# Matthew-Mosior/text-compression

Measured on AMD Instinct MI355X. Metric: BWT+MTF+RLE encode MB/s on 1 GiB ACGTN, higher is better.
Workload: dtype u8; 1 GPU; 1 x 1073741824-byte iid ACGTN record(s) (splitmix64 counter generator), fused BWT->MTF->RLE encode, in/out resident in HBM; record_bytes=1073741824, records=1, parallelism=record-per-gpu x1

## Files before the change

text-compression_amd/csrc/tc_msd.hpp:

```cpp
#pragma once
#include "tc_sa.hpp"

#ifndef MSD_NT
#define MSD_NT 1024
#endif
#ifndef MSD_ITEMS
#define MSD_ITEMS 8
#endif
#define MSD_TILE (MSD_NT * MSD_ITEMS)
#ifndef MSD_GROUP
#define MSD_GROUP 16
#endif
#define MSD_GLOG (MSD_GROUP == 32 ? 5 : MSD_GROUP == 16 ? 4 : 3)
#ifndef MSD_SUB
#define MSD_SUB 1
#endif
#ifndef MSD_BPC
#define MSD_BPC 1
#endif
#define MSD_LEVELS 3
#define MSDF_CAP_SMALL 2048
#ifndef MSDF_KO_NT
#define MSDF_KO_NT 256
#endif
// ... 274 lines not shown
                add(k0); add(k1); add(k2); add(k3);
            }
            for (; p < hi; p += MSD_NT) add(keys[p]);
        }
        __syncthreads();
        if (JOINT) {
            for (u32 w = tid; w < 32768; w += MSD_NT) {
                const u32 v = s_joint[w];
                if (v) {
                    atomicAdd(&joint_out[((size_t)sq * 256 + jr.dig[w >> 8]) * 256 + (w & 255u)], v);
                    atomicAdd(&s_cnt[jr.dig[w >> 8]], v);
                    s_joint[w] = 0;
                }
            }
            __syncthreads();
        }
        if (tid < 256) {
            L.seg[((size_t)sq + b) * 256 + tid] = s_cnt[tid];
            s_cnt[tid] = 0;
        }
    }
}

__global__ __launch_bounds__(256) void msd_scan_kernel(MsdLevel L, u32 G, u32 *maxchild) {
    __shared__ u32 s_scan[256 / 64 + 1];
    const u32 q = blockIdx.x, d = threadIdx.x;
    const u32 cnt = L.pcnt[q];
    const size_t c = (size_t)q * 256 + d;
    if (cnt == 0) {
        L.ccnt[c] = 0;
        L.cstart[c] = L.pstart[q];
        return;
    }
    if (L.aligned) {
        const u32 tot = L.cnt_in[c];
        u32 all;
        const u32 excl = block_excl_sum<256>(tot, s_scan, &all);
        const u32 start = L.pstart[q] + excl;
        L.cstart[c] = start;
        L.ccnt[c] = tot;
        L.seg[((size_t)q + msd_block_of_parent(L, q, G)) * 256 + d] = start;
        if (d == 0 && all != cnt) atomicOr(L.flags, 8u);
        if (maxchild) {
            u32 m = tot;
#pragma unroll
            for (int x = 32; x >= 1; x >>= 1) {
                const u32 o = __shfl_xor(m, x, 64);
                m = m > o ? m : o;
            }
            if ((d & 63) == 0 && m > MSDF_CAP_SMALL) atomicMax(maxchild, m);
        }
        return;
    }
    const u32 T = L.tpre[L.nparents];
    const u32 bf = msd_block_of_tile(T, L.tpre[q], G), bl = msd_block_of_tile(T, L.tpre[q + 1] - 1, G);
    u32 tot = 0;
#pragma unroll 8
    for (u32 b = bf; b <= bl; b++) {
        const u32 v = L.seg[((size_t)q + b) * 256 + d];
        tot += msd_tile_lo(T, b, G) < msd_tile_lo(T, b + 1, G) ? v : 0u;
    }
    u32 all;
    const u32 excl = block_excl_sum<256>(tot, s_scan, &all);
    u32 run = L.pstart[q] + excl;
    L.cstart[c] = run;
    L.ccnt[c] = tot;
#pragma unroll 8
    for (u32 b = bf; b <= bl; b++) {
        const size_t o = ((size_t)q + b) * 256 + d;
        const u32 v = L.seg[o];
        if (msd_tile_lo(T, b, G) >= msd_tile_lo(T, b + 1, G)) continue;
        L.seg[o] = run;
        run += v;
    }
    if (maxchild) {
        u32 m = tot;
#pragma unroll
        for (int x = 32; x >= 1; x >>= 1) {
            const u32 o = __shfl_xor(m, x, 64);
            m = m > o ? m : o;
        }
        if ((d & 63) == 0 && m > MSDF_CAP_SMALL) atomicMax(maxchild, m);
    }
}

typedef u32 msd_u32x4 __attribute__((ext_vector_type(4)));
template <bool KEYGEN, bool VALS = true>
__global__ __launch_bounds__(MSD_NT) void msd_partition_kernel(MsdLevel L, const u64 *kin, const u32 *vin,
                                                               u64 *kout, u32 *vout, const u8 *text,
                                                               RadixKeyGen kg) {
    __shared__ __attribute__((aligned(16))) u64 s_keys[MSD_TILE];
    __shared__ __attribute__((aligned(16))) u32 s_vals[VALS ? MSD_TILE : 4];
    __shared__ __attribute__((aligned(16))) u64 c_keys[256 * MSD_GROUP];
    __shared__ __attribute__((aligned(16))) u32 c_vals[VALS ? 256 * MSD_GROUP : 4];
    __shared__ u32 s_cnt[256 * MSD_SUB], s_dstart[256 * MSD_SUB], s_r[256], s_cur[256], s_ph[256];
    __shared__ u32 s_scan[16];
    __shared__ u64 s_lmask[4];
#ifdef MSD_PROFILE
    __shared__ u64 s_dbg[2];
    if (threadIdx.x == 0) { s_dbg[0] = 0; s_dbg[1] = 0; }
#endif
    __shared__ u16 s_live[256];
    __shared__ u16 s_klut[KEYGEN ? 256 : 1];
    constexpr bool KG_SPLIT = KEYGEN && !VALS && MSD_ITEMS == 8;
    __shared__ __attribute__((aligned(16))) u8 s_kr[KG_SPLIT ? MSD_TILE + 16 + 80 + 32 : 16];
    __shared__ __attribute__((aligned(16))) u8 s_kg8[KG_SPLIT ? MSD_TILE + 64 : 16];
    __shared__ u32 s_scan2[2];
    static_assert(MSD_GROUP == 8 || MSD_GROUP == 16 || MSD_GROUP == 32, "group = 8, 16 or 32 pairs");
    static_assert(((size_t)MSD_TILE * (VALS ? 12 : 8) + 256 * MSD_GROUP * (VALS ? 12 : 8) + 8192 + (KG_SPLIT ? 2 * MSD_TILE + 256 : 0)) * (VALS ? 1 : MSD_BPC) <= 163840, "LDS budget");
    __shared__ MsdTileInfo s_info[4];

    const u32 tid = threadIdx.x, G = gridDim.x, b = msd_logical_wg(blockIdx.x, G);
    if (KEYGEN && tid < 256) s_klut[tid] = kg.lut[tid];
    if (tid < 256) { s_r[tid] = 0; s_ph[tid] = 0; s_cur[tid] = 0; }
    for (u32 i = tid; i < 256 * MSD_SUB; i += MSD_NT) s_cnt[i] = 0;
    if (tid == 0) {
        u32 ta = 0, tb = 0;
        if (!(L.aligned && (*L.flags & 8u))) msd_block_range(L, b, G, &ta, &tb);
        s_scan2[0] = ta; s_scan2[1] = tb;
    }
    __syncthreads();
    const u32 t0 = s_scan2[0], t1 = s_scan2[1];
    if (t0 >= t1) return;
    MsdCur cs = {};
    if (tid == 0) {
        msd_cur_init(L, cs, t0);
        msd_cur_info(L, cs, t0, t1, &s_info[0]);
        msd_cur_info(L, cs, t0 + 1, t1, &s_info[1]);
        msd_cur_info(L, cs, t0 + 2, t1, &s_info[2]);
    }
    __syncthreads();

    constexpr int KG_PRE = 16, KG_SLOTS = MSD_TILE + KG_PRE + 80;
    u16 *k_c = reinterpret_cast<u16 *>(s_keys);
    u16 *k_g = k_c + KG_SLOTS;
    u8 *k_r = reinterpret_cast<u8 *>(k_g + KG_SLOTS);
    static_assert(KG_SLOTS * 5 <= MSD_TILE * 8, "key-generation image must fit under the staging keys");
    const u32 kg_units = KEYGEN ? (KG_PRE + MSD_TILE + kg.P * kg.s + kg.s + 15) / 16 : 0;

    u64 key[MSD_ITEMS];
    u32 val[MSD_ITEMS];
    msd_u32x4 raw = {0, 0, 0, 0}, nraw = {0, 0, 0, 0};
    auto kg_edge = [&](const MsdTileInfo ti) {
        return ti.base < (u32)KG_PRE || (u64)ti.base - KG_PRE + (u64)kg_units * 16 > (u64)kg.n_text ||
               ((((uintptr_t)text) + ti.base) & 15) != 0;
    };
    auto kg_load_plain = [&](const MsdTileInfo ti) {
        msd_u32x4 rw = {0, 0, 0, 0};
        if (tid < kg_units) {
            const i64 p0 = (i64)ti.base - KG_PRE + (i64)tid * 16;
            const i64 nt = (i64)kg.n_text;
            if (p0 >= 0 && p0 + 16 <= nt && ((((uintptr_t)text) + (u64)p0) & 15) == 0) {
                rw = *reinterpret_cast<const msd_u32x4 *>(text + p0);
            } else {
                u32 x[4] = {0, 0, 0, 0};
#pragma unroll 1
                for (int j = 0; j < 16; j++) {
                    const i64 pp = p0 + j;
                    const u32 c = (pp >= 0 && pp < nt) ? (u32)text[pp] : 0u;
                    x[j >> 2] |= c << (8 * (j & 3));
                }
                rw.x = x[0]; rw.y = x[1]; rw.z = x[2]; rw.w = x[3];
            }
        }
        return rw;
    };
// ... 933 lines not shown
```

text-compression_amd/csrc/tc_sa.hpp:

```cpp
#pragma once
#include <type_traits>
#include "tc_radix.hpp"

#define SA_NT 256
#define SA_ITEMS 16
#define SA_TILE (SA_NT * SA_ITEMS)
#define KB_HALO 72

struct SaConfig {
    u32 sigma_text;
    u32 B;
    u32 w;
    u32 s;
    u32 P;
    u32 h0;
    double entropy;
    u16 lut[256];
};

#ifdef __HIPCC__

__global__ __launch_bounds__(256) void hist256_kernel(const u8 *__restrict__ text, u64 n,
                                                      u32 *__restrict__ counts) {
    __shared__ u32 s_h[256 * 64];
// ... 899 lines not shown
            if (total == 0) return;
            if (l == 0) {
                abase = atomicAdd(&a.counters[0], total);
                atomicOr(&a.counters[1], 2u);
            }
            abase = __shfl(abase, 0, 64);
            if ((u64)abase + total > (u64)a.fix_cap) return;
        }
    }
}

__global__ __launch_bounds__(256) void finish_filter_kernel(u32 *__restrict__ slot, u32 count,
                                                            const u32 *__restrict__ ovbits, u32 *ndropped) {
    __shared__ u32 s_n;
    if (threadIdx.x == 0) s_n = 0;
    __syncthreads();
    u32 mine = 0;
    for (u64 k = (u64)blockIdx.x * 256 + threadIdx.x; k < count; k += (u64)gridDim.x * 256) {
        const u32 j = slot[k];
        if ((ovbits[j >> 5] >> (j & 31)) & 1u) {
            slot[k] = 0xFFFFFFFFu;
            mine++;
        }
    }
    for (int d = 32; d >= 1; d >>= 1) mine += (u32)__shfl_xor((int)mine, d, 64);
    if (lane_id() == 0 && mine) atomicAdd(&s_n, mine);
    __syncthreads();
    if (threadIdx.x == 0 && s_n) atomicAdd(ndropped, s_n);
}

__global__ __launch_bounds__(64) void finish_regions_kernel(const u32 *__restrict__ rcount, u32 rcap,
                                                            u32 *__restrict__ roff, u32 *__restrict__ counters) {
    const u32 l = threadIdx.x;
    const u32 c = rcount[l * FIN_RSTRIDE];
    const bool over = c > rcap;
    u32 inc = over ? rcap : c;
    const u32 mine = inc;
    for (int d = 1; d < 64; d <<= 1) {
        const u32 t = (u32)__shfl_up((int)inc, d, 64);
        if ((int)l >= d) inc += t;
    }
    roff[l] = inc - mine;
    const u64 anyover = __ballot(over);
    if (l == 63) {
        roff[64] = inc;
        counters[0] = anyover ? 0xFFFFFFF0u : inc;
    }
}
__global__ __launch_bounds__(256) void finish_compact_kernel(const u32 *__restrict__ roff, u32 rcap,
                                                             const u32 *__restrict__ in_slot,
                                                             const u32 *__restrict__ in_idx,
                                                             const u32 *__restrict__ in_grp,
                                                             u32 *__restrict__ out_slot, u32 *__restrict__ out_idx,
                                                             u32 *__restrict__ out_grp,
                                                             const u32 *__restrict__ in_x = nullptr, u32 *__restrict__ out_x = nullptr,
                                                             u32 x_cap = 0) {
    const u32 total = roff[64];
    for (u64 k = (u64)blockIdx.x * 256 + threadIdx.x; k < total; k += (u64)gridDim.x * 256) {
        u32 lo = 0, hi = FIN_REGIONS;
        while (hi - lo > 1) {
            const u32 mid = (lo + hi) >> 1;
            if (roff[mid] <= (u32)k) lo = mid; else hi = mid;
        }
        const u64 src = (u64)lo * rcap + ((u32)k - roff[lo]);
        out_slot[k] = in_slot[src];
        out_idx[k] = in_idx[src];
        out_grp[k] = in_grp[src];
        if (in_x && k < x_cap) out_x[k] = in_x[src];
    }
}

#define TP_SLOT_BITS 17
#define TP_BLOOM_LOG2 18
#define TP_MAX_TIED (1u << 15)
struct TiedTable {
    u64 *key;
    u32 *grp;
    u32 *cnt;
    u32 *bloom;
};
__device__ __forceinline__ u64 tp_mix(u64 v) { return v * 0x9E3779B97F4A7C15ull; }
__device__ __forceinline__ u32 tp_sym(u32 c) { return __umul24(c, 0x9E3779u); }
__device__ __forceinline__ u32 tp_rotl(u32 x, u32 r) { return __builtin_amdgcn_alignbit(x, x, (32u - r) & 31u); }

__global__ __launch_bounds__(256) void tied_table_kernel(const u32 *__restrict__ klo, const u32 *__restrict__ khi,
                                                         const u32 *__restrict__ grp, u32 m, u32 B, u32 sdig, u32 P,
                                                         TiedTable T) {
    const u32 k = blockIdx.x * 256 + threadIdx.x;
    if (k >= m) return;
    const u64 key56 = ((u64)khi[k] << 32) | klo[k];
    u64 v = 0;
    u32 H = 0;
    for (u32 f = 0; f < P; f++) {
        const u32 g = (u32)(key56 >> (48 - 8 * f)) & 255u;
        u32 div = 1;
        for (u32 j = 1; j < sdig; j++) div *= B;
        for (u32 j = 0; j < sdig; j++, div /= B) {
            const u32 c = (g / div) % B;
            v = v * B + c;
            H = tp_rotl(H, 1) ^ tp_sym(c);
        }
    }
    const u32 hb = H >> (32 - TP_BLOOM_LOG2);
    atomicOr(&T.bloom[hb >> 5], 1u << (hb & 31));
    u32 slot = (u32)(tp_mix(v) >> (64 - TP_SLOT_BITS));
    for (u32 probe = 0; probe < (1u << TP_SLOT_BITS); probe++) {
        const u64 old = atomicCAS((unsigned long long *)&T.key[slot], 0ull, (unsigned long long)v);
        if (old == 0ull || old == v) {
            T.grp[slot] = grp[k];
            return;
        }
        slot = (slot + 1) & ((1u << TP_SLOT_BITS) - 1u);
    }
}

#define TPK_NT 256
#define TPK_PER 64
#define TPK_TILE (TPK_NT * TPK_PER)
#define TPK_PAD(p) ((p) + ((p) >> 6) * 4u)
template <int S>
__global__ __launch_bounds__(TPK_NT) void tied_probe_kernel(const u8 *__restrict__ text, u32 n, RadixKeyGen kg,
                                                            TiedTable T, u32 *__restrict__ out_slot,
                                                            u32 *__restrict__ out_idx, u32 *__restrict__ out_grp,
                                                            u32 *total, u32 cap) {
    constexpr u32 h = 7 * S;
    constexpr int WD = (64 + h + 3) / 4;
    static_assert(h <= 56 && WD <= 30, "the window is 16 own dwords + at most 14 of the next thread's");
    __shared__ u32 s_bloom[(1u << TP_BLOOM_LOG2) / 32];
    __shared__ __attribute__((aligned(16))) u8 s_code[TPK_PAD(TPK_TILE + 64) + 16];
    __shared__ u8 s_lut[256];
    const u32 tid = threadIdx.x;
    const u32 B = kg.B;
    for (u32 i = tid; i < (1u << TP_BLOOM_LOG2) / 32; i += TPK_NT) s_bloom[i] = T.bloom[i];
    s_lut[tid] = (u8)kg.lut[tid];
    const u32 ntiles = (n + TPK_TILE - 1) / TPK_TILE;
    constexpr int NU = (TPK_TILE + 64 + TPK_NT * 16 - 1) / (TPK_NT * 16);
    uint4 raw[NU];
    auto unit_ok = [&](u32 base, int i) -> bool {
        const u32 p = ((u32)i * TPK_NT + tid) * 16;
        const u64 g = (u64)base + p;
        return p < TPK_TILE + 64 && g + 16 <= n && ((((uintptr_t)text) + g) & 15) == 0;
    };
    auto fetch = [&](u32 base) {
#pragma unroll
        for (int i = 0; i < NU; i++) {
            raw[i] = make_uint4(0, 0, 0, 0);
            if (unit_ok(base, i)) raw[i] = *reinterpret_cast<const uint4 *>(text + (u64)base + ((u32)i * TPK_NT + tid) * 16);
        }
    };
    if (blockIdx.x < ntiles) fetch(blockIdx.x * TPK_TILE);
    for (u32 tile = blockIdx.x; tile < ntiles; tile += gridDim.x) {
        const u32 base = tile * TPK_TILE;
        __syncthreads();
#pragma unroll
        for (int i = 0; i < NU; i++) {
            const u32 p = ((u32)i * TPK_NT + tid) * 16;
            if (p >= TPK_TILE + 64) continue;
            const u64 g = (u64)base + p;
            if (unit_ok(base, i)) {
                const u32 x[4] = {raw[i].x, raw[i].y, raw[i].z, raw[i].w};
#pragma unroll
                for (int j = 0; j < 16; j++) s_code[TPK_PAD(p + j)] = s_lut[(x[j >> 2] >> (8 * (j & 3))) & 255u];
            } else {
                for (int j = 0; j < 16; j++) s_code[TPK_PAD(p + j)] = g + j < n ? s_lut[text[g + j]] : (u8)0;
            }
        }
        if (tile + gridDim.x < ntiles) fetch((tile + gridDim.x) * TPK_TILE);
        lds_barrier();
        const u32 p0 = tid * TPK_PER;
        if (base + p0 < n) {
            u32 W[WD];
            {
                const u32 *own = reinterpret_cast<const u32 *>(s_code + 68u * tid);
                const u32 *nxt = reinterpret_cast<const u32 *>(s_code + 68u * (tid + 1));
#pragma unroll
                for (int i = 0; i < WD; i++) W[i] = i < 16 ? own[i] : nxt[i - 16];
            }
            auto code = [&](int x) -> u32 { return (W[x >> 2] >> (8 * (x & 3))) & 255u; };
            u32 H = 0;
#pragma unroll
            for (int j = 0; j < (int)h; j++) H = tp_rotl(H, 1) ^ tp_sym(code(j));
            u64 hits = 0;
#pragma unroll
            for (int j = 0; j < TPK_PER; j++) {
                const u32 hb = H >> (32 - TP_BLOOM_LOG2);
                hits |= (u64)((s_bloom[hb >> 5] >> (hb & 31)) & 1u) << j;
                H = tp_rotl(H, 1) ^ tp_rotl(tp_sym(code(j)), h & 31u) ^ tp_sym(code(j + (int)h));
            }
            while (hits) {
                const u32 j = (u32)__builtin_ctzll(hits);
                hits &= hits - 1;
                const u32 pos = base + p0 + j;
                if (pos >= n) break;
                u64 v = 0;
                for (u32 x = 0; x < h; x++) v = v * B + s_code[TPK_PAD(p0 + j + x)];
                u32 slot = (u32)(tp_mix(v) >> (64 - TP_SLOT_BITS));
                for (u32 probe = 0; probe < (1u << TP_SLOT_BITS); probe++) {
                    const u64 kk = T.key[slot];
                    if (kk == v) {
                        const u32 jj = atomicAdd(&T.cnt[slot], 1u);
                        const u32 o = atomicAdd(total, 1u);
                        if (o < cap) {
                            const u32 g0 = T.grp[slot];
                            out_slot[o] = g0 + jj;
                            out_idx[o] = pos;
                            out_grp[o] = g0;
                        }
                        break;
                    }
                    if (kk == 0ull) break;
                    slot = (slot + 1) & ((1u << TP_SLOT_BITS) - 1u);
                }
            }
        }
    }
}

__global__ __launch_bounds__(256) void pack_active_kernel(const u32 *__restrict__ slot,
                                                          const u32 *__restrict__ grp, u32 m,
                                                          u64 *__restrict__ keys) {
    u32 k = blockIdx.x * 256 + threadIdx.x;
    if (k < m) keys[k] = ((u64)slot[k] << 32) | grp[k];
}
__global__ __launch_bounds__(256) void unpack_active_kernel(const u64 *__restrict__ keys, u32 m,
                                                            u32 *__restrict__ slot,
                                                            u32 *__restrict__ grp) {
    u32 k = blockIdx.x * 256 + threadIdx.x;
    if (k < m) {
        slot[k] = (u32)(keys[k] >> 32);
        grp[k] = (u32)keys[k];
    }
}

struct RankLookup {
    const u32 *isa;
    const u32 *t_idx;
    const u32 *t_rank;
    u32 t_n;
    const u64 *skeys;
    const u64 *tkeys;
    int tshift;
    const u32 *sa;
    const u64 *t_bits;
    const u32 *t_dir;
    const u32 *kdir;
    int kdir_bits;
    const u8 *text;
    u32 n, N;
    u32 B, w, s, P;
    u32 h0;
    u16 lut[256];
};

__device__ __forceinline__ int suffix_cmp(const u8 *text, u32 n, u64 x, u64 y, u32 h) {
    for (u32 t = 0; t < h; t++, x++, y++) {
        int cx = x < n ? (int)text[x] : -1, cy = y < n ? (int)text[y] : -1;
        if (cx != cy) return cx < cy ? -1 : 1;
        if (cx < 0) return 0;
    }
    return 0;
}

template <bool WAVE = false>
__device__ __forceinline__ u32 rank_of(const RankLookup &r, const u16 *s_lut, u64 p) {
    if (p >= r.N) return 0u;
    if (r.isa) return r.isa[p];
    if (r.t_bits) {
        const u64 wbits = r.t_bits[p >> 6];
        if ((wbits >> (p & 63)) & 1ull)
            return r.t_rank[r.t_dir[p >> 6] + (u32)__popcll(wbits & ((1ull << (p & 63)) - 1ull))];
    } else {
        u32 lo = 0, hi = r.t_n;
        while (lo < hi) {
            u32 mid = (lo + hi) >> 1;
            if (r.t_idx[mid] < (u32)p) lo = mid + 1; else hi = mid;
        }
        if (lo < r.t_n && r.t_idx[lo] == (u32)p) return r.t_rank[lo];
    }
    u64 key = 0;
    if (p + 64 <= r.n && r.P * r.s <= 56) {
        u64 wv[7];
#pragma unroll
        for (int x = 0; x < 7; x++) __builtin_memcpy(&wv[x], r.text + p + 8 * x, 8);
        const u32 len = r.P * r.s;
        int sh = 64;
        u32 g = 0, t = 0;
#pragma unroll
        for (int k = 0; k < 56; k++) {
            if ((u32)k < len) {
                g = g * r.B + (u32)s_lut[(u32)(wv[k >> 3] >> (8 * (k & 7))) & 255u];
                if (++t == r.s) {
                    sh -= (int)r.w;
                    key |= (u64)g << sh;
                    g = 0; t = 0;
                }
            }
// ... 338 lines not shown
```

text-compression_amd/csrc/tc_sa_host.hpp:

```cpp
#pragma once
#include <chrono>

#include "tc_sa_plan.hpp"

#ifndef SA_KDIR_BITS
#define SA_KDIR_BITS 26
#endif
struct SaBuffers {
    u64 *k0, *k1;
    u32 *v0, *v1;
    u32 *isa;
    u32 *v2;
    u32 *act[2][4];
    u64 *sk[2];
    u32 *sv[2];
    u32 *t_idx, *t_rank;
    u64 *t_bits;
    u32 *t_dir;
    u32 *t_bsum;
    u32 *fin_rc;
    u32 *kdir;
    u64 sparse_cap;
    u32 *hist;
    u64 *rstatus;
// ... 9 lines not shown
};

static inline u64 msd_min_n() { return (u64)env_int("TC_SA_MSD_MIN_LOG2", 27) >= 40 ? ~0ull : 1ull << env_int("TC_SA_MSD_MIN_LOG2", 27); }
static inline bool msd_wanted(u64 N) { return env_int("TC_SA_MSD", 1) != 0 && N >= msd_min_n() && N > 4 * MSD_TILE; }

static size_t sa_carve(Arena &A, u64 N, SaBuffers &b, bool own_v1) {
    b.k0 = A.get<u64>(N);
    b.k1 = A.get<u64>(N);
    b.v0 = A.get<u32>(N);
    b.v1 = own_v1 ? A.get<u32>(N) : nullptr;
    b.isa = A.get<u32>(N + 1);
    b.v2 = A.get<u32>(N);
    b.sparse_cap = N / 8 + 1024;
    for (int s = 0; s < 2; s++) {
        for (int q = 0; q < 3; q++) b.act[s][q] = A.get<u32>(N);
        b.act[s][3] = A.get<u32>(b.sparse_cap);
        b.sk[s] = A.get<u64>(b.sparse_cap);
        b.sv[s] = A.get<u32>(b.sparse_cap);
    }
    b.t_idx = A.get<u32>(b.sparse_cap);
    b.t_rank = A.get<u32>(b.sparse_cap);
    b.t_bits = A.get<u64>(N / 64 + 2);
    b.t_dir = A.get<u32>(N / 64 + 2);
    b.t_bsum = A.get<u32>(N / 64 / BDIR_TILE + 2);
    b.fin_rc = A.get<u32>(FIN_REGIONS * FIN_RSTRIDE + 128);
    b.kdir = A.get<u32>(((size_t)1 << SA_KDIR_BITS) + 2 + ((size_t)1 << SA_KDIR_BITS) / KDF_CHUNK + 64);
    b.hist = A.get<u32>(RDX_MAX_PASSES * RDX_BINS);
    b.rstatus = A.get<u64>(radix_status_words(N));
    b.gstatus = A.get<u64>(2 * (size_t)tc_cdiv(N, GRP_TILE) + 4);
    b.counts = A.get<u32>(260);
    {
        SegBuffers &g = b.seg;
        g.cap_runs = (size_t)(N / SEG_CAP + 2);
        g.cap_tiles = (size_t)(N / SEG_PT + 2) + g.cap_runs;
        g.segbits = A.get<u64>(seg_bit_words(N));
        g.ybits = A.get<u64>(seg_bit_words(N));
        for (int q = 0; q < 2; q++) {
            g.lstart[q] = A.get<u32>(g.cap_runs);
            g.lsize[q] = A.get<u32>(g.cap_runs);
            g.ltbase[q] = A.get<u32>(g.cap_runs);
            g.lshift[q] = A.get<u32>(g.cap_runs);
        }
        g.tile_seg = A.get<u32>(g.cap_tiles);
        g.hist = A.get<u32>(g.cap_runs * 256);
        g.mm = A.get<u32>(g.cap_runs * 2);
        g.counters = A.get<u32>(64);
    }
    for (int l = 0; l <= MSD_LEVELS; l++) b.msd_pstart[l] = b.msd_pcnt[l] = nullptr;
    if (msd_wanted(N)) {
        b.msd_grid = 256 * MSD_BPC;
        size_t np = 1;
        for (int l = 0; l <= MSD_LEVELS; l++, np *= 256) {
            b.msd_pstart[l] = A.get<u32>(np);
            b.msd_pcnt[l] = A.get<u32>(np);
            if (l < MSD_LEVELS) {
                b.msd_tpre[l] = A.get<u32>(np + 1);
                b.msd_seg[l] = A.get<u32>((np + b.msd_grid) * 256);
            }
        }
        b.msd_joint = A.get<u32>((size_t)256 * 256 * 256);
        b.tp.key = A.get<u64>((size_t)1 << TP_SLOT_BITS);
        b.tp.grp = A.get<u32>((size_t)1 << TP_SLOT_BITS);
        b.tp.cnt = A.get<u32>((size_t)1 << TP_SLOT_BITS);
        b.tp.bloom = A.get<u32>(((size_t)1 << TP_BLOOM_LOG2) / 32);
    }
    b.chain_ref = A.get<u32>(N + 1);
    b.chain_code = A.get<u32>(N + 1);
    b.chain_summ = A.get<u32>(chain_summ_words());
    return A.off;
}

enum SaSlot {
    SA_SLOT_PRIMARY = 0,
    SA_SLOT_ACTIVE = 1,
    SA_SLOT_PROBE = 11,
    SA_SLOT_TIED = 12,
    SA_SLOT_DROPPED = 13,
    SA_SLOT_SAMPLE = 14,
    SA_SLOT_MAXCHILD = 15,
    SA_SLOT_SEG = 24,
    SA_SLOT_ERR = 62,
    SA_SLOT_MSD_PROF = 64,
    SA_SLOT_MSDK_PROF = 112,
};
static inline u32 sa_slot_lo(const tc_ctx *ctx, int slot) { return (u32)(ctx->h_scalars[slot] & 0xffffffffu); }
static inline u32 sa_slot_hi(const tc_ctx *ctx, int slot) { return (u32)(ctx->h_scalars[slot] >> 32); }
static inline u32 *sa_dev_slot(tc_ctx *ctx, int slot) { return reinterpret_cast<u32 *>(ctx->d_scalars + slot); }

#ifdef SEG_PROFILE
static void seg_profile_dump(tc_ctx *ctx, u32 m) {
    u64 h[16];
    TC_HIP(ctx, hipStreamSynchronize(ctx->stream));
    TC_HIP(ctx, hipMemcpyFromSymbol(h, HIP_SYMBOL(seg_prof), sizeof h));
    const double w = (double)(h[7] | 1);
    fprintf(stderr, "seg_small: %llu members, %llu windows (that sort), mid members per window %.0f | cycles per window: bits %.0f attr+masks %.0f (prefix) %.0f image %.0f tiny+compact %.0f tiny store %.0f network %.0f store %.0f\n",
            (unsigned long long)m, (unsigned long long)h[7], h[8] / w, h[0] / w, h[1] / w, 0.0, h[2] / w, h[3] / w, h[4] / w, h[5] / w, h[6] / w);
    memset(h, 0, sizeof h);
    TC_HIP(ctx, hipMemcpyToSymbol(HIP_SYMBOL(seg_prof), h, sizeof h));
}
#else
static inline void seg_profile_dump(tc_ctx *, u32) {}
#endif

static void seg_sort_pairs(tc_ctx *ctx, SegBuffers &g, u64 *kx, u32 *vx, u64 *ky, u32 *vy, u32 m, int rbits) {
    hipStream_t s = ctx->stream;
    const u32 nwords = (u32)seg_bit_words(m);
    TC_HIP(ctx, hipMemsetAsync(g.ybits, 0, (size_t)nwords * sizeof(u64), s));
    TC_HIP(ctx, hipMemsetAsync(g.counters, 0, 8 * sizeof(u32), s));
    u32 igrid = tc_cdiv((u64)nwords * 64, 256);
    if (igrid > 16384) igrid = 16384;
    seg_init_kernel<<<igrid, 256, 0, s>>>(kx, m, g.segbits, nwords, g.lstart[0], g.lsize[0], g.ltbase[0], g.lshift[0],
                                          (u32)(rbits > 8 ? rbits - 8 : 0), g.counters, (u32)g.cap_runs);
    TC_LAUNCH_CHECK(ctx);
    const int nlev = 8;
    int cur = 0;
    for (int L = 0;; L++) {
        TC_HIP(ctx, hipMemcpyAsync(&ctx->h_scalars[SA_SLOT_SEG], g.counters + 2 * cur, 2 * sizeof(u32), hipMemcpyDeviceToHost, s));
        TC_HIP(ctx, hipStreamSynchronize(s));
        const u32 S = sa_slot_lo(ctx, SA_SLOT_SEG), T = sa_slot_hi(ctx, SA_SLOT_SEG);
        if (S == 0) break;
        if (L >= nlev) TC_FAIL(ctx, TC_ERR_INTERNAL, "segmented sort: %u runs still unsorted after %d levels", S, nlev);
        if (S > g.cap_runs || T > g.cap_tiles) TC_FAIL(ctx, TC_ERR_INTERNAL, "segmented sort: %u long runs / %u tiles exceed the tables", S, T);
        const int nxt = cur ^ 1;
        TC_HIP(ctx, hipMemsetAsync(g.hist, 0, (size_t)S * 256 * sizeof(u32), s));
        seg_mm_init_kernel<<<tc_cdiv(S, 256), 256, 0, s>>>(g.mm, S);
        TC_LAUNCH_CHECK(ctx);
        TC_HIP(ctx, hipMemsetAsync(g.counters + 2 * nxt, 0, 2 * sizeof(u32), s));
        u32 wgrid = tc_cdiv(S, 4);
        if (wgrid > 8192) wgrid = 8192;
        seg_tilemap_kernel<<<wgrid, 256, 0, s>>>(g.lsize[cur], g.ltbase[cur], S, g.tile_seg, (u32)g.cap_tiles);
        TC_LAUNCH_CHECK(ctx);
        seg_count_kernel<<<T, 256, 0, s>>>(kx, ky, g.lstart[cur], g.lsize[cur], g.ltbase[cur], g.lshift[cur], g.tile_seg, g.counters + 2 * cur, g.hist, g.mm);
        TC_LAUNCH_CHECK(ctx);
        seg_scan_kernel<<<wgrid, 256, 0, s>>>(g.lstart[cur], g.lsize[cur], g.lshift[cur], g.counters + 2 * cur, g.hist, g.mm, g.segbits, 0,
                                              g.lstart[nxt], g.lsize[nxt], g.ltbase[nxt], g.lshift[nxt], g.counters + 2 * nxt, (u32)g.cap_runs);
        TC_LAUNCH_CHECK(ctx);
        seg_scatter_kernel<<<T, 256, 0, s>>>(kx, vx, ky, vy, g.lstart[cur], g.lsize[cur], g.ltbase[cur], g.lshift[cur], g.tile_seg, g.counters + 2 * cur,
                                             g.hist, g.mm, g.ybits);
        TC_LAUNCH_CHECK(ctx);
        cur = nxt;
    }
    seg_small_kernel<<<tc_cdiv(m, SEG_SPAN), SEG_NT, 0, s>>>(kx, vx, ky, vy, m, g.segbits, g.ybits);
    TC_LAUNCH_CHECK(ctx);
    seg_profile_dump(ctx, m);
}

static void sa_choose_config(const u32 *counts, u64 n, int forced_fields, SaConfig &c) {
    u32 sig = 0;
    double H = 0;
    for (int v = 0; v < 256; v++) {
        c.lut[v] = 0;
        if (counts[v]) {
            c.lut[v] = (u16)(++sig);
            double p = (double)counts[v] / (double)n;
            H -= p * log2(p);
        }
    }
    c.sigma_text = sig;
    c.B = sig + 1;
    if (c.B <= 16) {
        c.w = 8;
        c.s = 1;
        u32 pw = c.B;
        while (pw * c.B <= 256) {
            pw *= c.B;
            c.s++;
// ... 336 lines not shown
    fa.ovbits = b.act[1][0];
    tc_memset_async(ctx, ctx->d_scalars + SA_SLOT_TIED, 0, 2 * sizeof(u64));
    tc_memset_async(ctx, b.fin_rc, 0, (FIN_REGIONS * FIN_RSTRIDE + 128) * sizeof(u32));
}

static Round0Out sa_round0_lsd(SaRun &R, const Round0Plan &pl) {
    Round0Out o;
    o.msd = o.msd_big = o.keyonly = false;
    sa_round0_begin(R, pl.topbits, o);
    R.st().msd_path = 0;
    RadixPlan plan;
    plan.add_range(64 - pl.topbits, 64);
    RadixBuffers rb = sa_build_keys_and_sort(R, plan, true);
    o.npass = plan.npass;
    o.keys = rb.keys;
    o.fa.keys = rb.keys; o.fa.sa_in = rb.vals;
    const u32 waves = tc_cdiv(R.N, 64 * FIN_WPW);
    finish_kernel<<<tc_cdiv(waves, FIN_NT / 64), FIN_NT, 0, R.stream()>>>(o.fa);
    TC_LAUNCH_CHECK(R.ctx);
    return o;
}

static Round0Out sa_round0_msd(SaRun &R, const Round0Plan &pl, bool keyonly) {
    tc_ctx *ctx = R.ctx;
    SaBuffers &b = R.b;
    const SaConfig &cfg = R.cfg;
    hipStream_t s = R.stream();
    tc_stats &st = R.st();
    const u32 n = (u32)R.n, N = (u32)R.N;
    Round0Out o;
    o.msd = true; o.msd_big = pl.msd_big; o.keyonly = keyonly;
    sa_round0_begin(R, 8 * MSD_LEVELS, o);
    u32 *counters = o.fa.counters;
    RadixKeyGen kg = sa_keygen(R);
    radix_keygen_hash(kg);
    if (R.K.keygen_hash == 0) kg.hash_ok = 0;
    MsdTextDigit td;
    sa_fill(cfg, td);
    td.text = R.text; td.n = n;
    td.hash_ok = kg.hash_ok; td.hsh = kg.hsh; td.tlo = kg.tlo; td.thi = kg.thi;
    u32 G = b.msd_grid < (u32)ctx->num_cus * MSD_BPC ? b.msd_grid : (u32)ctx->num_cus * MSD_BPC;
    if (ctx->reserved_cus > 0 && G > (u32)(ctx->num_cus - ctx->reserved_cus) * MSD_BPC)
        G = (u32)(ctx->num_cus - ctx->reserved_cus) * MSD_BPC;
    if (R.K.msd_grid > 0 && (u32)R.K.msd_grid < G) G = (u32)R.K.msd_grid;
    u32 *maxchild = sa_dev_slot(ctx, SA_SLOT_MAXCHILD);
    msd_root_kernel<<<1, 1, 0, s>>>(b.msd_pstart[0], b.msd_pcnt[0], N, maxchild);
    TC_LAUNCH_CHECK(ctx);
    u64 *kbuf[2] = {b.k0, b.k1};
    u32 *vbuf[2] = {keyonly ? nullptr : b.v0, keyonly ? nullptr : R.sa};
    st.msd_keyonly = keyonly ? 1u : 0u;
    ctx->pev_used = 0;
    st.keygen_fused = 1;
    MsdJointRows jr;
    u32 nrows = 0;
    {
        memset(jr.row, 0xff, sizeof jr.row);
        memset(jr.dig, 0, sizeof jr.dig);
        u32 nd = 1;
        for (u32 j = 0; j < cfg.s; j++) nd *= cfg.B;
        for (u32 d = 0; d < nd && d < 256; d++) {
            bool real = true;
            for (u32 v = d, j = 0; j < cfg.s; j++, v /= cfg.B) real = real && (v % cfg.B) != 0;
            if (real) {
                if (nrows < 128) { jr.row[d] = (u8)nrows; jr.dig[nrows] = (u8)d; }
                nrows++;
            }
        }
    }
    const bool joint = R.K.msd_joint != 0 && nrows <= 128;
    if (joint) tc_memset_async(ctx, b.msd_joint, 0, (size_t)256 * 256 * 256 * sizeof(u32));
    u32 np = 1;
    for (int l = 0; l < MSD_LEVELS; l++, np *= 256) {
        MsdLevel ML;
        ML.pstart = b.msd_pstart[l]; ML.pcnt = b.msd_pcnt[l]; ML.tpre = b.msd_tpre[l];
        ML.nparents = np; ML.shift = 56 - 8 * l; ML.seg = b.msd_seg[l];
        ML.cstart = b.msd_pstart[l + 1]; ML.ccnt = b.msd_pcnt[l + 1];
        ML.aligned = (joint && l == MSD_LEVELS - 1) ? 1 : 0;
        ML.ntot = N; ML.cnt_in = b.msd_joint; ML.flags = counters + 1;
        ML.dbg = ctx->d_scalars + SA_SLOT_MSD_PROF + 16 * l;
        const u64 *kin = l ? kbuf[(l - 1) & 1] : nullptr;
        const u32 *vin = l ? vbuf[(l - 1) & 1] : nullptr;
        msd_prep_kernel<<<1, 1024, 0, s>>>(ML.pcnt, np, b.msd_tpre[l]);
        TC_LAUNCH_CHECK(ctx);
        if (l == 0) msd_count_kernel<true, false><<<G, MSD_NT, 0, s>>>(ML, nullptr, td, nullptr, jr);
        else if (ML.aligned) {  }
        else if (joint && l == MSD_LEVELS - 2) msd_count_kernel<false, true><<<G, MSD_NT, 0, s>>>(ML, kin, td, b.msd_joint, jr);
        else msd_count_kernel<false, false><<<G, MSD_NT, 0, s>>>(ML, kin, td, nullptr, jr);
        TC_LAUNCH_CHECK(ctx);
        msd_scan_kernel<<<np, 256, 0, s>>>(ML, G, l == MSD_LEVELS - 1 ? maxchild : nullptr);
        TC_LAUNCH_CHECK(ctx);
        const bool ev = ctx->profile && ctx->pev_used < 16;
        if (ev) TC_HIP(ctx, hipEventRecord(ctx->pev[2 * ctx->pev_used], s));
        if (keyonly) {
            if (l == 0) msd_partition_kernel<true, false><<<G, MSD_NT, 0, s>>>(ML, nullptr, nullptr, kbuf[0], nullptr, R.text, kg);
            else msd_partition_kernel<false, false><<<G, MSD_NT, 0, s>>>(ML, kin, nullptr, kbuf[l & 1], nullptr, R.text, kg);
        } else if (l == 0) msd_partition_kernel<true><<<G, MSD_NT, 0, s>>>(ML, nullptr, nullptr, kbuf[0], vbuf[0], R.text, kg);
        else msd_partition_kernel<false><<<G, MSD_NT, 0, s>>>(ML, kin, vin, kbuf[l & 1], vbuf[l & 1], R.text, kg);
        TC_LAUNCH_CHECK(ctx);
        if (ev) {
            TC_HIP(ctx, hipEventRecord(ctx->pev[2 * ctx->pev_used + 1], s));
            ctx->pev_used++;
        }
    }
    o.keys = kbuf[(MSD_LEVELS - 1) & 1];
    MsdFinishArgs mf;
    mf.keys = o.keys; mf.vals = vbuf[(MSD_LEVELS - 1) & 1];
    mf.pcnt = b.msd_pcnt[MSD_LEVELS - 1];
    mf.cstart = b.msd_pstart[MSD_LEVELS]; mf.ccnt = b.msd_pcnt[MSD_LEVELS];
    mf.sa_out = R.sa; mf.L = R.d_L;
    mf.out_slot = o.fa.out_slot; mf.out_idx = o.fa.out_idx; mf.out_grp = o.fa.out_grp;
    mf.rcount = o.fa.rcount; mf.rcap = o.fa.rcap; mf.counters = counters;
    mf.kout = kbuf[MSD_LEVELS & 1];
    o.keys_sorted = mf.kout;
    mf.whole_list = b.msd_seg[MSD_LEVELS - 1];
    mf.whole_cap = 1u << 20;
    mf.out_khi = b.v0;
    MsdFinishLut *flut = reinterpret_cast<MsdFinishLut *>(b.msd_seg[MSD_LEVELS - 1] + 2 * (size_t)mf.whole_cap);
    msd_finish_lut_kernel<<<1, 256, 0, s>>>(b.msd_pcnt[1], flut);
    TC_LAUNCH_CHECK(ctx);
    mf.lut = R.K.msd_finish_lut != 0 ? flut : nullptr;
    if (pl.msd_big && keyonly) {
        msd_finish_kernel<MSDF_BIG_NT, MSDF_BIG_ITEMS, 1, 5, true, false><<<np / 256, MSDF_BIG_NT, 0, s>>>(mf);
    } else if (pl.msd_big) {
        msd_finish_kernel<MSDF_BIG_NT, MSDF_BIG_ITEMS, 1, 5, true><<<np / 256, MSDF_BIG_NT, 0, s>>>(mf);
        TC_LAUNCH_CHECK(ctx);
        msd_whole_kernel<<<1024, MSDW_NT, 0, s>>>(mf);
    } else if (keyonly && R.K.msd_finish_ko != 0) {
        msd_finish_ko_kernel<3><<<np / 256, 256, 0, s>>>(mf, flut);
        msdk_profile_dump(ctx);
    } else if (keyonly) {
        msd_finish_kernel<MSDF_KO_NT, MSDF_CAP_SMALL / MSDF_KO_NT, 4, 1, false, false><<<np / 256, MSDF_KO_NT, 0, s>>>(mf);
    } else {
        msd_finish_kernel<256, 8, 4, 1, false><<<np / 256, 256, 0, s>>>(mf);
    }
    TC_LAUNCH_CHECK(ctx);
    o.npass = MSD_LEVELS;
    st.msd_path = 1;
    msd_profile_dump(ctx);
    return o;
}

static bool sa_keyonly_recover(SaRun &R, u32 fm, u32 flags) {
    tc_ctx *ctx = R.ctx;
    SaBuffers &b = R.b;
    const SaConfig &cfg = R.cfg;
    hipStream_t s = R.stream();
    const u32 n = (u32)R.n;
    bool ok = fm <= TP_MAX_TIED && (u64)fm + 1024 <= b.sparse_cap && !(flags & 2u);
    if (ok) sa_trace_tied_checksums(R, fm);
    if (ok && fm > 0) {
        tc_memset_async(ctx, b.tp.key, 0, sizeof(u64) << TP_SLOT_BITS);
        tc_memset_async(ctx, b.tp.cnt, 0, sizeof(u32) << TP_SLOT_BITS);
        tc_memset_async(ctx, b.tp.bloom, 0, ((size_t)1 << TP_BLOOM_LOG2) / 8);
        u32 *d_total = sa_dev_slot(ctx, SA_SLOT_PROBE);
        tc_memset_async(ctx, d_total, 0, sizeof(u64));
        tied_table_kernel<<<tc_cdiv(fm, 256), 256, 0, s>>>(b.act[0][1], b.act[0][3], b.act[0][2], fm, cfg.B, cfg.s, cfg.P, b.tp);
        TC_LAUNCH_CHECK(ctx);
        const RadixKeyGen kgp = sa_keygen(R);
        u32 pgrid = (u32)ctx->num_cus * 3;
        if (pgrid > tc_cdiv(n, TPK_TILE)) pgrid = tc_cdiv(n, TPK_TILE);
        switch (cfg.s) {
#define TC_PROBE(S) case S: tied_probe_kernel<S><<<pgrid, TPK_NT, 0, s>>>(R.text, n, kgp, b.tp, b.act[0][0], b.act[0][1], b.act[0][2], d_total, fm); break;
            TC_PROBE(1) TC_PROBE(2) TC_PROBE(3) TC_PROBE(4) TC_PROBE(5) TC_PROBE(6) TC_PROBE(7) TC_PROBE(8)
#undef TC_PROBE
            default: TC_FAIL(ctx, TC_ERR_INTERNAL, "key-only levels: %u symbols per field", cfg.s);
        }
        TC_LAUNCH_CHECK(ctx);
        tc_d2h(ctx, &ctx->h_scalars[SA_SLOT_PROBE], ctx->d_scalars + SA_SLOT_PROBE, sizeof(u64));
        TC_HIP(ctx, hipStreamSynchronize(s));
        ok = sa_slot_lo(ctx, SA_SLOT_PROBE) == fm;
    }
    if (R.K.trace)
        fprintf(stderr, "textcomp: key-only levels: %u tied suffixes %s (the pass over the text met %u)\n", fm,
                ok ? "found again in the text" : "-- NOT recoverable: the levels run again with suffix starts", sa_slot_lo(ctx, SA_SLOT_PROBE));
    return ok;
}

static void sa_tier2_fix(SaRun &R, const FinishArgs &fa, u32 &fm, u32 &flags, u32 &fm_dropped) {
    tc_ctx *ctx = R.ctx;
    hipStream_t s = R.stream();
    const u32 fm_lean = fm;
    u32 *flagword = sa_dev_slot(ctx, SA_SLOT_TIED) + 1;
    u32 *ndropped = sa_dev_slot(ctx, SA_SLOT_DROPPED);
    tc_memset_async(ctx, flagword, 0, sizeof(u32));
    tc_memset_async(ctx, ndropped, 0, sizeof(u64));
    tc_memset_async(ctx, fa.ovbits, 0, ((size_t)tc_cdiv(R.N, 64) + 1) * sizeof(u64));
    const u32 fwaves = tc_cdiv(R.N, 64 * FIX_WIN);
    finish_fix_kernel<<<tc_cdiv(fwaves, FIN_NT / 64), FIN_NT, 0, s>>>(fa);
    TC_LAUNCH_CHECK(ctx);
    if (fm_lean) {
        finish_filter_kernel<<<tc_cdiv(fm_lean, 256) < 4096u ? tc_cdiv(fm_lean, 256) : 4096u, 256, 0, s>>>(fa.out_slot, fm_lean, fa.ovbits, ndropped);
        TC_LAUNCH_CHECK(ctx);
    }
    tc_d2h(ctx, &ctx->h_scalars[SA_SLOT_TIED], ctx->d_scalars + SA_SLOT_TIED, 2 * sizeof(u64));
    TC_HIP(ctx, hipStreamSynchronize(s));
    fm = sa_slot_lo(ctx, SA_SLOT_TIED);
    flags = sa_slot_hi(ctx, SA_SLOT_TIED);
    fm_dropped = sa_slot_lo(ctx, SA_SLOT_DROPPED);
}

static void sa_order_tied(SaRun &R, u32 fm, u32 slot_bits) {
    tc_ctx *ctx = R.ctx;
    SaBuffers &b = R.b;
    hipStream_t s = R.stream();
    if (fm <= SEG_W && R.K.tiny != 0) {
        tied_small_kernel<0><<<1, SEG_NT, 0, s>>>(b.act[0][0], b.act[0][1], b.act[0][2], fm, nullptr, nullptr, nullptr);
        TC_LAUNCH_CHECK(ctx);
        return;
    }
    pack_active_kernel<<<tc_cdiv(fm, 256), 256, 0, s>>>(b.act[0][0], b.act[0][2], fm, b.sk[0]);
    TC_LAUNCH_CHECK(ctx);
    TC_HIP(ctx, hipMemcpyAsync(b.sv[0], b.act[0][1], fm * sizeof(u32), hipMemcpyDeviceToDevice, s));
    RadixPlan ps;
    ps.add_range(32, 32 + (int)slot_bits);
    RadixBuffers rs = sa_sparse_buffers(R);
    radix_sort_pairs(ctx, rs, fm, ps, false, false);
    unpack_active_kernel<<<tc_cdiv(fm, 256), 256, 0, s>>>(rs.keys, fm, b.act[0][0], b.act[0][2]);
    TC_LAUNCH_CHECK(ctx);
    TC_HIP(ctx, hipMemcpyAsync(b.act[0][1], rs.vals, fm * sizeof(u32), hipMemcpyDeviceToDevice, s));
}

static void sa_key_round(SaRun &R, u64 *kall) {
    tc_ctx *ctx = R.ctx;
    SaBuffers &b = R.b;
    hipStream_t s = R.stream();
    tc_stats &st = R.st();
    const u32 mm = (u32)R.m;
    key_round_kernel<<<tc_cdiv(mm, 256), 256, 0, s>>>(b.act[0][0], b.act[0][2], kall, mm, b.sk[0], b.sv[0]);
    TC_LAUNCH_CHECK(ctx);
    seg_sort_pairs(ctx, b.seg, b.sk[0], b.sv[0], b.sk[1], b.sv[1], mm, 32);
    key_round_store_kernel<<<tc_cdiv(mm, 256), 256, 0, s>>>(b.sk[0], b.act[0][0], mm, kall);
    TC_LAUNCH_CHECK(ctx);
    GroupArgs gk = {};
    gk.keys = b.sk[0]; gk.count = mm; gk.vals = b.sv[0]; gk.vals_are_idx = 0; gk.norank = 1;
    gk.in_slot = b.act[0][0]; gk.in_idx = b.act[0][1];
    gk.out_slot = b.act[1][0]; gk.out_idx = b.act[1][1]; gk.out_grp = b.act[1][2];
    sa_run_group(R, false, gk);
    const u64 m2 = sa_fetch_m(R);
    for (int q = 0; q < 3; q++)
        if (m2) TC_HIP(ctx, hipMemcpyAsync(b.act[0][q], b.act[1][q], m2 * sizeof(u32), hipMemcpyDeviceToDevice, s));
    st.m[st.rounds] = R.m; st.key_bytes[st.rounds] = 8; st.passes[st.rounds] = 1; st.h[st.rounds] = (u32)R.h_start;
    st.rounds++;
    st.seg_rounds++;
    if (R.K.trace)
        fprintf(stderr, "textcomp: key round: %u members of whole buckets ordered by the key's remaining 32 bits, %llu stay tied\n", mm, (unsigned long long)m2);
    R.m = m2;
    R.h_start = R.cfg.h0;
}

enum Round0Result {
    R0_ACCEPTED,
    R0_GIVE_WAY,
// ... 384 lines not shown
```

Before: 53550 MB/s.

## Use two-bit bloom filter for tied probe and dedicated root-level MSD scan

The tied-suffix bloom filter now sets two bits inside one word per hash instead of a single bit, so the probe kernel rejects more false positives before entering the slow hash-table path. The first MSD level's scan is replaced by a root-specific kernel with one block per digit. Each block sums tile counts with vectorised loads and writes segment offsets, with the level-0 count kernel redirected to a separate seg buffer. A compile-time-gated profiling counter for the probe is also added. The trade-off is a denser bloom filter and an extra count buffer.

Result: no change. 54040 MB/s, median of 6 (+0.9%).

```diff
diff --git a/text-compression_amd/csrc/tc_msd.hpp b/text-compression_amd/csrc/tc_msd.hpp
--- a/text-compression_amd/csrc/tc_msd.hpp
+++ b/text-compression_amd/csrc/tc_msd.hpp
@@ -380,6 +380,39 @@
         }
         if ((d & 63) == 0 && m > MSDF_CAP_SMALL) atomicMax(maxchild, m);
     }
+}
+
+__global__ __launch_bounds__(256) void msd_scan_root_kernel(MsdLevel L, const u32 *__restrict__ cnt, u32 G) {
+    __shared__ u32 s_scan[256 / 64 + 1];
+    const u32 d = blockIdx.x, tid = threadIdx.x;
+    const u32 T = L.tpre[1];
+    auto owns = [&](u32 b) { return b < G && msd_tile_lo(T, b, G) < msd_tile_lo(T, b + 1, G); };
+    u32 mine = 0;
+    for (u32 b = tid; b < G; b += 256) {
+        if (!owns(b)) continue;
+        const u32 *row = cnt + (size_t)b * 256;
+        const uint4 *rv = reinterpret_cast<const uint4 *>(row);
+#pragma unroll 16
+        for (u32 j = 0; j < (d >> 2); j++) {
+            const uint4 x = rv[j];
+            mine += x.x + x.y + x.z + x.w;
+        }
+        for (u32 j = d & ~3u; j < d; j++) mine += row[j];
+    }
+    u32 before;
+    block_excl_sum<256>(mine, s_scan, &before);
+    u32 run = L.pstart[0] + before;
+    if (tid == 0) L.cstart[d] = run;
+    for (u32 b0 = 0; b0 < G; b0 += 256) {
+        const u32 b = b0 + tid;
+        const bool own = owns(b);
+        const u32 v = own ? cnt[(size_t)b * 256 + d] : 0u;
+        u32 all;
+        const u32 excl = block_excl_sum<256>(v, s_scan, &all);
+        if (own) L.seg[(size_t)b * 256 + d] = run + excl;
+        run += all;
+    }
+    if (tid == 0) L.ccnt[d] = run - (L.pstart[0] + before);
 }
 
 typedef u32 msd_u32x4 __attribute__((ext_vector_type(4)));
diff --git a/text-compression_amd/csrc/tc_sa.hpp b/text-compression_amd/csrc/tc_sa.hpp
--- a/text-compression_amd/csrc/tc_sa.hpp
+++ b/text-compression_amd/csrc/tc_sa.hpp
@@ -1005,6 +1005,9 @@
 __device__ __forceinline__ u64 tp_mix(u64 v) { return v * 0x9E3779B97F4A7C15ull; }
 __device__ __forceinline__ u32 tp_sym(u32 c) { return __umul24(c, 0x9E3779u); }
 __device__ __forceinline__ u32 tp_rotl(u32 x, u32 r) { return __builtin_amdgcn_alignbit(x, x, (32u - r) & 31u); }
+static_assert(TP_BLOOM_LOG2 == 18, "tp_bloom_*: 13 bits of word index, two 5-bit bit indices");
+__device__ __forceinline__ u32 tp_bloom_word(u32 H) { return H >> 19; }
+__device__ __forceinline__ u32 tp_bloom_mask(u32 H) { return (1u << ((H >> 14) & 31u)) | (1u << ((H >> 9) & 31u)); }
 
 __global__ __launch_bounds__(256) void tied_table_kernel(const u32 *__restrict__ klo, const u32 *__restrict__ khi,
                                                          const u32 *__restrict__ grp, u32 m, u32 B, u32 sdig, u32 P,
@@ -1024,8 +1027,7 @@
             H = tp_rotl(H, 1) ^ tp_sym(c);
         }
     }
-    const u32 hb = H >> (32 - TP_BLOOM_LOG2);
-    atomicOr(&T.bloom[hb >> 5], 1u << (hb & 31));
+    atomicOr(&T.bloom[tp_bloom_word(H)], tp_bloom_mask(H));
     u32 slot = (u32)(tp_mix(v) >> (64 - TP_SLOT_BITS));
     for (u32 probe = 0; probe < (1u << TP_SLOT_BITS); probe++) {
         const u64 old = atomicCAS((unsigned long long *)&T.key[slot], 0ull, (unsigned long long)v);
@@ -1106,11 +1108,17 @@
             u64 hits = 0;
 #pragma unroll
             for (int j = 0; j < TPK_PER; j++) {
-                const u32 hb = H >> (32 - TP_BLOOM_LOG2);
-                hits |= (u64)((s_bloom[hb >> 5] >> (hb & 31)) & 1u) << j;
+                const u32 bw = s_bloom[tp_bloom_word(H)];
+                hits |= (u64)((bw >> ((H >> 14) & 31u)) & (bw >> ((H >> 9) & 31u)) & 1u) << j;
                 H = tp_rotl(H, 1) ^ tp_rotl(tp_sym(code(j)), h & 31u) ^ tp_sym(code(j + (int)h));
             }
+#ifdef TPK_PROFILE
+            u32 pf_pass = (u32)__popcll(hits), pf_turns = 0, pf_found = 0;
+#endif
             while (hits) {
+#ifdef TPK_PROFILE
+                pf_turns++;
+#endif
                 const u32 j = (u32)__builtin_ctzll(hits);
                 hits &= hits - 1;
                 const u32 pos = base + p0 + j;
@@ -1123,6 +1131,9 @@
                     if (kk == v) {
                         const u32 jj = atomicAdd(&T.cnt[slot], 1u);
                         const u32 o = atomicAdd(total, 1u);
+#ifdef TPK_PROFILE
+                        pf_found++;
+#endif
                         if (o < cap) {
                             const u32 g0 = T.grp[slot];
                             out_slot[o] = g0 + jj;
@@ -1135,6 +1146,20 @@
                     slot = (slot + 1) & ((1u << TP_SLOT_BITS) - 1u);
                 }
             }
+#ifdef TPK_PROFILE
+            {
+                u64 *dbg = reinterpret_cast<u64 *>(total) - 11 + 124;
+                u32 mt = pf_turns;
+#pragma unroll
+                for (int x = 32; x >= 1; x >>= 1) {
+                    const u32 o = __shfl_xor(mt, x, 64);
+                    mt = mt > o ? mt : o;
+                }
+                if (pf_pass) atomicAdd((unsigned long long *)&dbg[0], (unsigned long long)pf_pass);
+                if (pf_found) atomicAdd((unsigned long long *)&dbg[1], (unsigned long long)pf_found);
+                if ((tid & 63) == 0 && mt) atomicAdd((unsigned long long *)&dbg[2], (unsigned long long)mt);
+            }
+#endif
         }
     }
 }
diff --git a/text-compression_amd/csrc/tc_sa_host.hpp b/text-compression_amd/csrc/tc_sa_host.hpp
--- a/text-compression_amd/csrc/tc_sa_host.hpp
+++ b/text-compression_amd/csrc/tc_sa_host.hpp
@@ -115,6 +115,7 @@
     SA_SLOT_ERR = 62,
     SA_SLOT_MSD_PROF = 64,
     SA_SLOT_MSDK_PROF = 112,
+    SA_SLOT_TPK_PROF = 124,
 };
 static inline u32 sa_slot_lo(const tc_ctx *ctx, int slot) { return (u32)(ctx->h_scalars[slot] & 0xffffffffu); }
 static inline u32 sa_slot_hi(const tc_ctx *ctx, int slot) { return (u32)(ctx->h_scalars[slot] >> 32); }
@@ -617,12 +618,16 @@
         const u32 *vin = l ? vbuf[(l - 1) & 1] : nullptr;
         msd_prep_kernel<<<1, 1024, 0, s>>>(ML.pcnt, np, b.msd_tpre[l]);
         TC_LAUNCH_CHECK(ctx);
-        if (l == 0) msd_count_kernel<true, false><<<G, MSD_NT, 0, s>>>(ML, nullptr, td, nullptr, jr);
-        else if (ML.aligned) {  }
+        if (l == 0) {
+            MsdLevel MC = ML;
+            MC.seg = b.msd_seg[1];
+            msd_count_kernel<true, false><<<G, MSD_NT, 0, s>>>(MC, nullptr, td, nullptr, jr);
+        } else if (ML.aligned) {  }
         else if (joint && l == MSD_LEVELS - 2) msd_count_kernel<false, true><<<G, MSD_NT, 0, s>>>(ML, kin, td, b.msd_joint, jr);
         else msd_count_kernel<false, false><<<G, MSD_NT, 0, s>>>(ML, kin, td, nullptr, jr);
         TC_LAUNCH_CHECK(ctx);
-        msd_scan_kernel<<<np, 256, 0, s>>>(ML, G, l == MSD_LEVELS - 1 ? maxchild : nullptr);
+        if (l == 0) msd_scan_root_kernel<<<256, 256, 0, s>>>(ML, b.msd_seg[1], G);
+        else msd_scan_kernel<<<np, 256, 0, s>>>(ML, G, l == MSD_LEVELS - 1 ? maxchild : nullptr);
         TC_LAUNCH_CHECK(ctx);
         const bool ev = ctx->profile && ctx->pev_used < 16;
         if (ev) TC_HIP(ctx, hipEventRecord(ctx->pev[2 * ctx->pev_used], s));
@@ -703,6 +708,17 @@
         TC_LAUNCH_CHECK(ctx);
         tc_d2h(ctx, &ctx->h_scalars[SA_SLOT_PROBE], ctx->d_scalars + SA_SLOT_PROBE, sizeof(u64));
         TC_HIP(ctx, hipStreamSynchronize(s));
+#ifdef TPK_PROFILE
+        {
+            u64 h[3];
+            tc_d2h(ctx, h, ctx->d_scalars + SA_SLOT_TPK_PROF, sizeof h);
+            TC_HIP(ctx, hipStreamSynchronize(s));
+            fprintf(stderr, "tied probe: %u members, %llu positions passed the filter, %llu found in the table, %llu slow-path turns over all waves (%.1f per wave and tile)\n",
+                    fm, (unsigned long long)h[0], (unsigned long long)h[1], (unsigned long long)h[2],
+                    (double)h[2] / ((double)tc_cdiv(n, TPK_TILE) * (TPK_NT / 64)));
+            tc_memset_async(ctx, ctx->d_scalars + SA_SLOT_TPK_PROF, 0, sizeof h);
+        }
+#endif
         ok = sa_slot_lo(ctx, SA_SLOT_PROBE) == fm;
     }
     if (R.K.trace)
```
